# ETH3D/dataset-pipeline

Hardware: AMD Instinct MI355X
Metric: ICP correspondences/sec (higher is better)
Workload: dtype f32 (f64 accumulation); 1 GPU; ICPScanAligner 2 scans x 50000000 points, -d 0.01 (BASELINE.json configs[1] shape), one outer iteration per step; scans=2, parallelism=dp1

## Files before the change

dataset-pipeline_amd/csrc/e3d_icp.hip:

```cpp
#include <atomic>
#include <algorithm>
#include <cfloat>
#include <chrono>
#include <cmath>
#include <condition_variable>
#include <cstdio>
#include <functional>
#include <map>
#include <memory>
#include <mutex>
#include <thread>

#include "../../include/e3d_hip.h"
#include "e3d_comm.hpp"
#include "e3d_icp_kernels.hpp"
#include "e3d_math.hpp"

#pragma clang fp contract(off)

namespace e3d {

static thread_local std::string g_last_error;
void set_last_error(const std::string& msg) { g_last_error = msg; }
const char* last_error_cstr() { return g_last_error.c_str(); }

int require_device() {
  int n = 0;
  if (hipGetDeviceCount(&n) != hipSuccess || n <= 0) throw Error(E3D_ERR_NO_DEVICE, "no HIP device visible (libe3dhip needs an MI355X / gfx950 GPU)");
  return n;
}

struct IcpSwitches {
  int nn_mode = [] { const int v = env_int("E3D_NN_MODE", 0); return (v >= 0 && v <= 5) ? v : 0; }();
  int half = env_int("E3D_NN_HALF", 1);
  bool occupancy = env_default_on("E3D_NN_PRUNE");
  size_t dense_cells = [] { const char* e = getenv("E3D_DENSE_CELLS"); return e ? (size_t)strtoull(e, nullptr, 10) : (size_t)1 << 33; }();
  bool use_cert = env_default_on("E3D_NN_CERT");
  bool cert_skip = env_default_on("E3D_NN_CERT_SKIP");
  bool per_query = env_default_on("E3D_NN_PERQUERY");
  bool want_stats = env_default_off("E3D_NN_STATS");
  bool nn_profile = env_default_off("E3D_NN_PROFILE");
  double margin_frac = env_double("E3D_NN_MARGIN", 0.08), near_frac = env_double("E3D_NN_NEAR", 0.4);
  double np_frac = env_double("E3D_NN_NP_EXTRA", 0.5), np_gate = env_double("E3D_NN_NP_GATE", 0.2);
  size_t prune_min_list = (size_t)env_double("E3D_NN_PRUNE_MIN", 262144.0);
  long long far_div = [] { const char* e = getenv("E3D_NN_FAR_DIV"); return e ? atoll(e) : 32ll; }();
  bool fuse_update = env_default_on("E3D_NN_FUSE_UPDATE");
  double fuse_gate = env_double("E3D_NN_FUSE_GATE", 0.003);
  bool far_batch = env_default_on("E3D_NN_FAR_BATCH");
  bool seed_allowed = env_default_on("E3D_NN_SEED");
  double seed_frac = env_double("E3D_NN_SEED_FRAC", 0.3), seed_near = env_double("E3D_NN_SEED_NEAR", 0.4);
  bool seed_fresh = env_double("E3D_NN_SEED_FRESH", 0.0) != 0.0;
  bool batching = env_default_on("E3D_ICP_BATCH");
  int batch_mode = env_int("E3D_ICP_BATCH", 2);
  bool resident = env_default_on("E3D_ICP_RESIDENT");
  bool sequential_dsum = env_default_off("E3D_ICP_SEQUENTIAL_DISTANCE_SUM");
  bool lm_profile = env_default_off("E3D_LM_PROFILE");
  bool lm_trace = getenv("E3D_LM_TRACE") != nullptr;
  int solve_threads = env_int("E3D_LM_SOLVE_THREADS", 4);
  bool speculate = env_default_on("E3D_LM_SPECULATE");
  int spec_offset = env_int("E3D_LM_SPEC_OFFSET", 0);
};
static const IcpSwitches& icp_switches() { static const IcpSwitches sw; return sw; }

static int g_device = 0;
static int g_nn_mode = icp_switches().nn_mode;
static std::atomic<unsigned long long> g_grid_generation{0};

struct Cloud {
  size_t n = 0;
  bool fixed = false;
  DevBuf<float> raw_xyz, raw_nrm;
  float T[12] = {1, 0, 0, 0, 0, 1, 0, 0, 0, 0, 1, 0};
  bool grid_valid = false;
  float grid_radius = -1.f;
  float grid_T[12];
  DevBuf<float4> L4, LN, G4;
  DevBuf<HashEntry> table;
  DevBuf<unsigned> dense_start;
  bool has_dense = false;
  DevBuf<unsigned long long> half_prefix;
// ... 617 lines not shown
  NnPhase(hipStream_t st, int sl) : s(st), slot(sl) { if (icp_switches().nn_profile) { (void)hipStreamSynchronize(s); t0 = std::chrono::steady_clock::now(); } }
  ~NnPhase() { if (icp_switches().nn_profile) { (void)hipStreamSynchronize(s); g_nn_prof[slot] += std::chrono::duration<double, std::milli>(std::chrono::steady_clock::now() - t0).count(); } }
};
static void print_nn_profile(size_t n_pairs) {
  if (!icp_switches().nn_profile) return;
  fprintf(stderr, "[nn profile] certify + bounded search %.1f ms, keys + sort %.1f ms, match scan + compaction (+ plane growth) %.1f ms, %zu pairs\n",
          g_nn_prof[0], g_nn_prof[1], g_nn_prof[2], n_pairs);
  for (double& v : g_nn_prof) v = 0;
}

static bool pair_is_dense(const e3d_icp* h, const Cloud& tgt) {
  return h->nn_mode >= 2 || (h->nn_mode == 0 && (double)tgt.n >= 4.0 * (double)std::max(tgt.n_cells, 1u));
}
static bool pair_uses_rows(const e3d_icp* h, const Cloud& tgt) {
  return pair_is_dense(h, tgt) && tgt.has_dense && (h->nn_mode == 0 || h->nn_mode == 3 || h->nn_mode == 5);
}
static bool far_list_is_short(size_t n_far, size_t n) {
  const long long div = icp_switches().far_div;
  return n_far > 0 && (div <= 0 || n_far * (size_t)div < n);
}
static size_t resident_rows_cap(size_t n) { return div_up(n, 64) * 64; }
static size_t resident_bytes(size_t n) { return resident_rows_cap(n) * 24 + n * 4 + div_up(n, 64) * 4; }
static size_t source_view_cap(size_t n) { return resident_rows_cap(n) + 64; }
static size_t source_view_bytes(size_t n) { return source_view_cap(n) * 24; }
static bool alloc_trace() { static const bool on = [] { const char* e = getenv("E3D_ALLOC_TRACE"); return e && e[0] == '1'; }(); return on; }

struct BatchItem {
  PairJob* job; Cloud* src; Cloud* tgt; size_t j0, n; PairState* ps;
  InvMap im; CertParams cert; BoundParams bp; double cum_pair;
  MotionBound cum_up;
  float near2; bool none_near;
  bool certified = false, from_state = false; size_t n_near = 0, n_far = 0;
  bool rows_reset = false;
};

static void certify_ran(BatchItem& it, const unsigned* todo_len) {
  it.n_near = todo_len[0]; it.n_far = todo_len[1];
  it.ps->settled_frac = it.n ? 1.0 - (double)(it.n_near + it.n_far) / (double)it.n : 1.0;
  it.ps->certify_motion = it.src->last_motion + it.tgt->last_motion;
}

static void prepare_pair(BatchItem& it, float d) {
  const IcpSwitches& sw = icp_switches();
  const Cloud& src = *it.src; const Cloud& tgt = *it.tgt;
  const PairState& ps = *it.ps;
  it.im = make_invmap(tgt);
  it.cum_pair = src.cum_motion + tgt.cum_motion;
  MotionBound m_lo;
  pair_motion_bounds(ps, src, tgt, m_lo, it.cum_up);
  it.cert = make_cert_params(tgt, m_lo);
  it.n_far = it.n; it.n_near = 0;
  it.certified = !ps.fresh && sw.use_cert && certify_now(ps, src, tgt);
  it.from_state = !ps.fresh && sw.use_cert && !it.certified;
  it.near2 = (float)((sw.near_frac * (double)d) * (sw.near_frac * (double)d));
  it.none_near = sw.np_frac > 0 && (src.last_motion + tgt.last_motion) < sw.np_gate * (double)d;
  double smin = cloud_smin(tgt);
  if (!(smin > 1e-12)) smin = 1e-12;
  double m_local = 0;
  for (int k = 0; k < 3; ++k) m_local = std::max(m_local, std::max(std::fabs((double)tgt.lmin[k]), std::fabs((double)tgt.lmax[k])));
  it.bp.margin = (float)(sw.margin_frac * (double)d);
  it.bp.rho_scale = round_up_f((1.0 + 1e-5) / smin);
  it.bp.rho_pad = round_up_f(2.0 * tgt.build_slack + 8.0 * FLT_EPSILON * m_local);
  it.bp.lo = it.cert.lo;
  it.bp.cell_scale = it.cert.cell_scale; it.bp.cell_sub = it.cert.cell_sub;
  it.bp.np_extra = it.none_near ? (float)(sw.np_frac * (double)d) : 0.f;
}
// ... 6 lines not shown
  const unsigned long long* half = tgt.has_half ? tgt.half_prefix.p : nullptr;
  h->tm_bounded.start(s);
  launch_nn_bounded(srcG, todo_near, it.n_near, tgt.G4.p, tgt.dense_start.p, half, h->nn_mode == 5, tgt.grid, it.im, tgt.qrange, radius_sq(d), it.bp,
                    ps.match.p, ps.match2.p, match_d2, ps.lbe.p, s);
  if (far_list_is_short(it.n_far, it.n)) {
    launch_nn_bounded(srcG, todo_far, it.n_far, tgt.G4.p, tgt.dense_start.p, half, h->nn_mode == 5, tgt.grid, it.im, tgt.qrange, radius_sq(d), it.bp,
                      ps.match.p, ps.match2.p, match_d2, ps.lbe.p, s);
    it.n_near += it.n_far; it.n_far = 0;
  }
  h->tm_bounded.stop(s);
  if (it.n_near > 0) { rec.nn_bounded_launches++; rec.nn_bounded_queries += (long long)it.n_near; rec.nn_kernel_launches++; }
}

static void search_far_list(e3d_icp* h, BatchItem& it, const unsigned* list, float* match_d2, float d, EventTimer* nn_timer, e3d_icp_iter_record& rec) {
  hipStream_t s = h->stream;
  PairState& ps = *it.ps;
  const float4* srcG = it.src->G4.p + it.j0;
  size_t n_rows = 0;
  if (it.n_far > 0) {
    NnPhase ph(s, 1);
    n_rows = sort_query_keys_pruned(h, ps, *it.tgt, srcG, list, it.n_far, it.im, radius_sq(d), it.cert, match_d2, it.from_state);
    rec.nn_sort_calls++; rec.nn_kernel_launches++;
  }
  if (nn_timer) nn_timer->start(s);
  if (n_rows == 0) return;
  if (!nn_timer) h->tm_search.start(s);
  launch_rows(3, *it.tgt, srcG, h->vals_b.p, n_rows, it.im, radius_sq(d), it.cert, ps.match.p, match_d2, ps.lbe.p, ps.match2.p, s);
  if (!nn_timer) h->tm_search.stop(s);
  rec.nn_search_launches++; rec.nn_search_queries += (long long)n_rows; rec.nn_kernel_launches++;
}

static void print_pair_stats(const BatchItem& it) {
  if (!icp_switches().want_stats) return;
  fprintf(stderr, "[nn %d->%d] queries %zu bounded %zu rows %zu cum %.3g (last %.3g) err %.3g\n", it.job->src, it.job->tgt, it.n, it.n_near, it.n_far,
          it.cum_pair, it.src->last_motion + it.tgt->last_motion, it.src->err_max + it.tgt->err_max);
}

struct RowFrames { bool sg, tg; bool reset; };
static void ensure_source_view(Cloud& c, bool global, hipStream_t s) {
  const size_t cap = source_view_cap(c.n);
  bool valid = c.view_valid && c.V0.cap >= cap && c.V1.cap >= cap && c.view_gen == c.generation && c.view_global == global;
  if (valid && global && std::memcmp(c.view_T, c.T, sizeof c.view_T) != 0) valid = false;
  if (valid) return;
  if (alloc_trace() && (c.V0.cap < cap || c.V1.cap < cap))
    fprintf(stderr, "[rows] source view of cloud %d: %zu points, %zu bytes (%s frame)\n", c.cloud_index, c.n, source_view_bytes(c.n), global ? "global" : "local");
  c.V0.reserve(cap); c.V1.reserve(cap);
  launch_source_view(global ? c.G4.p : c.L4.p, c.LN.p, c.n, cap, global, to_affine(c.T), c.V0.p, c.V1.p, s);
  c.view_valid = true; c.view_global = global; c.view_gen = c.generation;
  std::memcpy(c.view_T, c.T, sizeof c.view_T);
}
static RowFrames ensure_resident_rows(PairState& ps, Cloud& src, const Cloud& tgt, size_t n, hipStream_t s) {
  const size_t cap = resident_rows_cap(n);
  const bool sg = src.fixed || src.cloud_index == 0, tg = tgt.fixed || tgt.cloud_index == 0;
  ensure_source_view(src, sg, s);
  bool valid = ps.rows_valid && ps.r0.cap >= cap && ps.r1.cap >= cap && ps.src_global == sg && ps.tgt_global == tg;
  if (valid && sg && std::memcmp(ps.src_T, src.T, sizeof ps.src_T) != 0) valid = false;
  if (valid && tg && std::memcmp(ps.tgt_T, tgt.T, sizeof ps.tgt_T) != 0) valid = false;
  if (!valid) {
    ps.r0.reserve(cap); ps.r1.reserve(cap); ps.plane_match.reserve(n); ps.glist.reserve(div_up(n, 64));
    E3D_HIP(hipMemsetAsync(ps.plane_match.p, 0xFE, sizeof(int) * n, s));
    if (cap > n) {
      E3D_HIP(hipMemsetAsync(ps.r0.p + n, 0xFF, sizeof(float2) * (cap - n), s));
      E3D_HIP(hipMemsetAsync(ps.r1.p + n, 0, sizeof(float4) * (cap - n), s));
    }
    ps.src_global = sg; ps.tgt_global = tg;
    std::memcpy(ps.src_T, src.T, sizeof ps.src_T); std::memcpy(ps.tgt_T, tgt.T, sizeof ps.tgt_T);
    ps.rows_valid = true;
  }
// ... 224 lines not shown
    prepare_pair(it, d);
    const RowFrames rf = ensure_resident_rows(ps, src, tgt, n, s);
    const bool tg = rf.tg;
    it.rows_reset = rf.reset;
    NnPairDev& P = T.pair[i];
    P.Gsrc = src.G4.p + it.j0; P.Gtgt = tgt.G4.p; P.S = tgt.dense_start.p; P.H8 = tgt.half_prefix.p;
    P.match = ps.match.p; P.match2 = ps.match2.p; P.lbe = ps.lbe.p; P.match_d2 = sl.match_d2.p;
    P.todo_near = sl.todo_near.p; P.todo_far = sl.todo_far.p; P.counts = h->d_todo_all.p + 2 * i;
    P.n = (unsigned)n; P.none_near = it.none_near ? 1 : 0;
    P.cum_up = it.cum_up; P.near2 = it.near2;
    P.g = tgt.grid; P.im = it.im; P.qr = tgt.qrange; P.bp = it.bp;
    P.Ptgt = tg ? tgt.G4.p : tgt.L4.p; P.LNtgt = tgt.LN.p;
    P.tgt_global = tg ? 1 : 0; P.Ttgt = to_affine(tgt.T);
    P.R0 = ps.r0.p; P.R1 = ps.r1.p; P.plane_match = ps.plane_match.p; P.glist = ps.glist.p;
    if (it.certified) { cert_blocks += (unsigned)div_up(n, (size_t)kNnCertBlockQueries); cert_queries += (long long)n; }
    T.cert_end[i] = cert_blocks;
    const unsigned nb = (unsigned)div_up(n, kBlock);
    upd_blocks += nb; T.upd_end[i] = upd_blocks;
    chunks += (unsigned)div_up((size_t)nb, (size_t)kNnScanChunk); T.chunk_end[i] = chunks;
  }
  h->block_counts.reserve(upd_blocks); h->block_d2.reserve(upd_blocks); h->block_groups.reserve(upd_blocks);
  h->chunk_sum.reserve(chunks + 1); h->chunk_d2.reserve(chunks + 1); h->chunk_groups.reserve(chunks + 1); h->chunk_rewritten.reserve(chunks + 1);
  {
    if (sw.fuse_update && cert_blocks) { h->block_done.reserve(upd_blocks); E3D_HIP(hipMemsetAsync(h->block_done.p, 0, upd_blocks, s)); }
    unsigned b0 = 0;
    for (size_t i = 0; i < B; ++i) {
      NnPairDev& P = T.pair[i];
      const bool on = sw.fuse_update && cert_blocks && items[i].certified && !items[i].rows_reset && (1.0 - items[i].ps->settled_frac) < sw.fuse_gate;
      P.upd_counts = on ? h->block_counts.p + b0 : nullptr; P.upd_d2 = on ? h->block_d2.p + b0 : nullptr;
      P.upd_groups = on ? h->block_groups.p + b0 : nullptr; P.upd_done = on ? h->block_done.p + b0 : nullptr;
      b0 = T.upd_end[i];
    }
  }
  E3D_HIP(hipMemcpyAsync(h->d_batch.p, h->h_batch.p, sizeof(NnBatchDev), hipMemcpyHostToDevice, s));
  if (cert_blocks) {
    h->tm_certify.start(s);
    launch_nn_certify_multi(h->d_batch.p, cert_blocks, radius_sq(d), s);
    h->tm_certify.stop(s);
    rec.nn_certify_launches++; rec.nn_certify_queries += cert_queries; rec.nn_kernel_launches++;
    copy_out(h->h_todo_all.p, h->d_todo_all.p, 2 * sizeof(unsigned) * B, s);
  }
  sync(h);
  unsigned job_blocks = 0;
  long long job_queries = 0;
  auto add_job = [&](size_t i, const unsigned* list, size_t n_list) {
    if (!n_list) return;
    const int jb = T.n_jobs++;
    T.job_pair[jb] = (int)i; T.job_list[jb] = list; T.job_n[jb] = (unsigned)n_list;
    job_blocks += (unsigned)div_up(n_list, kBlock); T.job_end[jb] = job_blocks;
    job_queries += (long long)n_list;
  };
  for (size_t i = 0; i < B; ++i) {
    BatchItem& it = items[i];
    if (!it.certified) continue;
    e3d_icp::PairSlot& sl = *h->slots[i];
    certify_ran(it, h->h_todo_all.p + 2 * i);
    add_job(i, sl.todo_near.p, it.n_near);
    if (far_list_is_short(it.n_far, it.n)) {
      add_job(i, sl.todo_far.p, it.n_far);
      it.n_near += it.n_far; it.n_far = 0;
    }
  }
  auto launch_bounded_jobs = [&] {
    if (T.n_jobs <= 0) return;
    E3D_HIP(hipMemcpyAsync(h->d_batch.p, h->h_batch.p, sizeof(NnBatchDev), hipMemcpyHostToDevice, s));
    h->tm_bounded.start(s);
    launch_nn_bounded_half_multi(h->d_batch.p, job_blocks, radius_sq(d), s);
    h->tm_bounded.stop(s);
    rec.nn_bounded_launches++; rec.nn_bounded_queries += job_queries; rec.nn_kernel_launches++;
  };
  auto seeds_for = [&](const BatchItem& it) { return sw.seed_allowed && it.n_far > 0 && (it.ps->fresh ? sw.seed_fresh : it.ps->matched_frac >= sw.seed_frac); };
  size_t far_pairs = 0, far_total = 0;
  int kb_max = 1;
  for (size_t i = 0; i < B; ++i) if (items[i].n_far > 0) { ++far_pairs; far_total += items[i].n_far; kb_max = std::max(kb_max, items[i].tgt->key_bits); }
  int pair_bits = 0;
  while (((size_t)1 << pair_bits) < B) ++pair_bits;
  const bool far_multi = sw.far_batch && far_pairs > 0 && (kb_max + pair_bits <= 32 || kb_max > 31) && kb_max + pair_bits <= 63;
  if (!far_multi) launch_bounded_jobs();
  if (far_multi) {
    const bool k32 = kb_max <= 31 && kb_max + pair_bits <= 32;
    bool seed_any = false;
    for (size_t i = 0; i < B; ++i)
      if (seeds_for(items[i])) seed_any = true;
    const size_t key_block = seed_any ? (size_t)kQuerySeedBlock : (size_t)kQueryKeysBlock;
    unsigned key_blocks = 0;
    for (size_t i = 0; i < B; ++i) {
      BatchItem& it = items[i];
      NnPairDev& P = T.pair[i];
      P.far_n = 0; P.far_list = nullptr; P.far_flags = 0; P.occ = nullptr; P.occ_stride = 0; P.rows_off = 0; P.rows_n = 0; P.seed_list = nullptr; P.seed2 = 0.f;
      if (it.n_far > 0) {
// ... 932 lines not shown
```

dataset-pipeline_amd/csrc/e3d_icp_certify.hip:

```cpp
#include <cstdlib>

#include "e3d_icp_device.hpp"

#pragma clang fp contract(off)

namespace e3d {

constexpr int kCertPerWave = 512;
template <int kCertUnroll>
__device__ __forceinline__ void nn_certify_body(const unsigned bx, const float4* __restrict__ Gsrc, size_t n, const float4* __restrict__ Gtgt,
                                                const MotionBound cum_up, float r2, float near2, int none_near, int* __restrict__ match,
                                                int* __restrict__ match2, const float* __restrict__ lbe,
                                                float* __restrict__ match_d2, unsigned* __restrict__ todo_near,
                                                unsigned* __restrict__ todo_far, unsigned* __restrict__ counts,
                                                unsigned* __restrict__ upd_counts = nullptr, double* __restrict__ upd_d2 = nullptr,
                                                unsigned* __restrict__ upd_groups = nullptr, unsigned char* __restrict__ upd_done = nullptr) {
  __shared__ unsigned s_list[2][kBlock / kWave][kCertPerWave];
  __shared__ unsigned s_cnt[2][kBlock / kWave];
  __shared__ unsigned s_base[2];
  const int lane = threadIdx.x & 63, w = threadIdx.x >> 6;
  const size_t j0 = ((size_t)bx * (kBlock / kWave) + (size_t)w) * kCertPerWave;
  unsigned cn = 0, cf = 0;
  for (int step0 = 0; step0 < kCertPerWave / kWave; step0 += kCertUnroll) {
    size_t jj[kCertUnroll];
    bool vv[kCertUnroll];
    int mm[kCertUnroll], mm2[kCertUnroll];
    float ll[kCertUnroll];
    float4 qq[kCertUnroll], c1[kCertUnroll], c2v[kCertUnroll];
#pragma unroll
    for (int u = 0; u < kCertUnroll; ++u) {
      jj[u] = j0 + (size_t)(step0 + u) * kWave + (size_t)lane;
      vv[u] = jj[u] < n;
      const size_t js = vv[u] ? jj[u] : 0;
      mm[u] = ld_stream(match + js); mm2[u] = ld_stream(match2 + js); ll[u] = ld_stream(lbe + js); qq[u] = ld_stream(Gsrc + js);
    }
#pragma unroll
    for (int u = 0; u < kCertUnroll; ++u) {
      c1[u] = Gtgt[mm[u] >= 0 ? mm[u] : 0];
      c2v[u] = Gtgt[(mm[u] >= 0 && mm2[u] >= 0) ? mm2[u] : 0];
    }
    unsigned ub_c = 0, ub_g = 0, ub_gm = 0;
    double ub_t = 0.0;
    bool ub_bad = false;
    static_assert(kCertUnroll == 4, "four steps of 64 queries = one block of the row update");
#pragma unroll
    for (int u = 0; u < kCertUnroll; ++u) {
    const size_t j = jj[u];
    const bool valid = vv[u];
    bool ok = false, near = false;
    bool swapped = false;
    float v_ok = 0.f;
    if (valid) {
      const float thr = (ll[u] - motion_up(qq[u], cum_up)) * 0.999999f;
      const float lim = thr * thr * 0.999999f;
      const int m = mm[u];
      if (m >= 0) {
        const int m2 = mm2[u];
        const float4 q = qq[u];
        const float4 c = c1[u];
        float v = sqdist_l2(q.x, q.y, q.z, c.x, c.y, c.z);
        if (m2 >= 0) {
          const float4 c2 = c2v[u];
          const float v2 = sqdist_l2(q.x, q.y, q.z, c2.x, c2.y, c2.z);
          if (v2 < v || (v2 == v && __float_as_uint(c2.w) < __float_as_uint(c.w))) {
            v = v2;
            if (thr > 0.f && v < lim && v < r2) { match[j] = m2; match2[j] = m; swapped = true; }
          }
        }
        ok = (thr > 0.f) && (v < lim) && (v < r2);
        near = v < near2;
        if (ok) { st_stream(match_d2 + j, v); v_ok = v; }
      } else {
        ok = (thr > 0.f) && (lim >= r2);
        near = none_near != 0;
        st_stream(match_d2 + j, r2);
      }
    }
    const unsigned long long fn = __ballot(valid && !ok && near), ff = __ballot(valid && !ok && !near);
    const unsigned long long below = (1ull << lane) - 1ull;
    if (valid && !ok) {
      if (near) s_list[0][w][cn + (unsigned)__popcll(fn & below)] = (unsigned)j;
      else s_list[1][w][cf + (unsigned)__popcll(ff & below)] = (unsigned)j | (mm[u] < 0 ? kListNoPartner : 0u);
    }
    cn += (unsigned)__popcll(fn); cf += (unsigned)__popcll(ff);
    if (upd_done) {
      const bool f = valid && mm[u] >= 0;
      const unsigned gc = (unsigned)__popcll(__ballot(f));
      const double gd = wave_sum((f && ok) ? (double)v_ok : 0.0);
      ub_c += gc; ub_t += gd;
      if (gc) { ++ub_g; ub_gm |= 1u << u; }
      if (__ballot(valid && (!ok || swapped))) ub_bad = true;
    }
    }
    if (upd_done) {
      const size_t blk = j0 / kBlock + (size_t)(step0 / kCertUnroll);
      if (blk < (n + kBlock - 1) / kBlock && lane == 0) {
        if (!ub_bad) { upd_counts[blk] = ub_c; upd_d2[blk] = ub_t; upd_groups[blk] = ub_g | (ub_gm << 8); }
        upd_done[blk] = ub_bad ? 0 : 1;
      }
    }
  }
  if (lane == 0) { s_cnt[0][w] = cn; s_cnt[1][w] = cf; }
  __syncthreads();
  if (threadIdx.x < 2) {
    unsigned tot = 0;
    for (int k = 0; k < kBlock / kWave; ++k) tot += s_cnt[threadIdx.x][k];
    s_base[threadIdx.x] = tot ? atomicAdd(&counts[threadIdx.x], tot) : 0u;
  }
  __syncthreads();
  unsigned bn = s_base[0], bf = s_base[1];
  for (int k = 0; k < w; ++k) { bn += s_cnt[0][k]; bf += s_cnt[1][k]; }
  for (unsigned i = (unsigned)lane; i < cn; i += kWave) todo_near[bn + i] = s_list[0][w][i];
  for (unsigned i = (unsigned)lane; i < cf; i += kWave) todo_far[bf + i] = s_list[1][w][i];
}

template <int kCertUnroll>
__global__ __launch_bounds__(kBlock) void k_nn_certify(const float4* __restrict__ Gsrc, size_t n, const float4* __restrict__ Gtgt,
                                                       MotionBound cum_up, float r2, float near2, int none_near, int* __restrict__ match,
                                                       int* __restrict__ match2, const float* __restrict__ lbe,
                                                       float* __restrict__ match_d2, unsigned* __restrict__ todo_near,
                                                       unsigned* __restrict__ todo_far, unsigned* __restrict__ counts) {
  nn_certify_body<kCertUnroll>(blockIdx.x, Gsrc, n, Gtgt, cum_up, r2, near2, none_near, match, match2, lbe, match_d2, todo_near, todo_far, counts);
}

__global__ __launch_bounds__(kBlock) void k_nn_certify_multi(const NnBatchDev* __restrict__ B, float r2) {
  const int p = nn_find_range(B->cert_end, B->n_pairs, blockIdx.x);
  const unsigned bx = blockIdx.x - (p ? B->cert_end[p - 1] : 0u);
  const NnPairDev& P = B->pair[p];
  nn_certify_body<4>(bx, P.Gsrc, (size_t)P.n, P.Gtgt, P.cum_up, r2, P.near2, P.none_near, P.match, P.match2, P.lbe, P.match_d2,
                     P.todo_near, P.todo_far, P.counts, P.upd_counts, P.upd_d2, P.upd_groups, P.upd_done);
}

template <int LPQ>
__global__ __launch_bounds__(kBlock) void k_nn_bounded(const float4* __restrict__ Gsrc, const unsigned* __restrict__ list,
                                                       unsigned n_list, const float4* __restrict__ Gtgt, const unsigned* __restrict__ S,
                                                       GridDesc g, InvMap im, QueryRange qr, float r2, BoundParams bp,
                                                       int* __restrict__ match, int* __restrict__ match2,
                                                       float* __restrict__ match_d2, float* __restrict__ lbe) {
  const unsigned i = (blockIdx.x * blockDim.x + threadIdx.x) / LPQ;
  const int sub = threadIdx.x % LPQ;
  if (i >= n_list) return;
  const unsigned j = list[i] & kListIndexMask;
  const float4 q = Gsrc[j];
  const int m = match[j];
  float d1 = r2;
  if (m >= 0) {
// ... 73 lines not shown
  }
  if (sub != 0) return;
  tie = (bd == bd2 && bd < kInf) || (bd2 == b3 && bd2 < kInf);
  if (tie) {
    bd = kInf; bd2 = kInf; b3 = kInf; bpos = -1; bpos2 = -1;
    unsigned boi = 0u, boi2 = 0u;
    for (int cz = z0; cz <= z1; ++cz) {
      for (int cy = y0; cy <= y1; ++cy) {
        const size_t row = ((size_t)cz * qr.D[1] + (size_t)cy) * qr.D[0];
        const unsigned s0 = S[row + (size_t)x0], s1 = S[row + (size_t)x1 + 1];
        for (unsigned p = s0; p < s1; ++p) {
          const float4 c = Gtgt[p];
          const float d2 = sqdist_l2(q.x, q.y, q.z, c.x, c.y, c.z);
          const unsigned oi = __float_as_uint(c.w);
          if (d2 < bd || (d2 == bd && oi < boi)) {
            b3 = fminf(b3, bd2); bd2 = bd; boi2 = boi; bpos2 = bpos; bd = d2; boi = oi; bpos = (int)p;
          } else if (d2 < bd2 || (d2 == bd2 && oi < boi2)) {
            b3 = fminf(b3, bd2); bd2 = d2; boi2 = oi; bpos2 = (int)p;
          } else {
            b3 = fminf(b3, d2);
          }
        }
      }
    }
  }
  const bool has1 = bd < r2, has2 = bd2 < r2;
  match[j] = has1 ? bpos : -1;
  match2[j] = has2 ? bpos2 : -1;
  match_d2[j] = has1 ? bd : r2;
  const float others2 = has2 ? b3 : (has1 ? bd2 : bd);
  lbe[j] = sqrtf(fminf(others2, cover_all2)) * 0.999999f + motion_lo(q, bp.lo);
}

constexpr int kHalfRuns = 18;
template <int BATCH>
__device__ __forceinline__ void nn_bounded_half_body(const unsigned bx, const float4* __restrict__ Gsrc, const unsigned* __restrict__ list,
                                                     unsigned n_list, const float4* __restrict__ Gtgt, const unsigned* __restrict__ S,
                                                     const unsigned long long* __restrict__ H8,
                                                     const GridDesc& g, const InvMap& im, const QueryRange& qr, float r2, const BoundParams& bp,
                                                     int* __restrict__ match, int* __restrict__ match2,
                                                     float* __restrict__ match_d2, float* __restrict__ lbe) {
  __shared__ unsigned s_runs[kHalfRuns][kBlock];
  __shared__ unsigned char s_len[kHalfRuns][kBlock];
  const unsigned i = bx * blockDim.x + threadIdx.x;
  if (i >= n_list) return;
  const unsigned j = list[i] & kListIndexMask;
  const float4 q = Gsrc[j];
  const int m = match[j];
  float d1 = r2;
  if (m >= 0) {
    const float4 pc = Gtgt[m];
    d1 = sqdist_l2(q.x, q.y, q.z, pc.x, pc.y, pc.z);
    const int m2 = match2[j];
    if (m2 >= 0) { const float4 pc2 = Gtgt[m2]; d1 = fminf(d1, sqdist_l2(q.x, q.y, q.z, pc2.x, pc2.y, pc2.z)); }
  }
  const float dr = sqrtf(fminf(d1, r2)) + ((m < 0) ? bp.np_extra : bp.margin);
  const float cover2 = (d1 < r2) ? fminf(dr * dr * 1.000001f, r2) : ((m < 0) ? dr * dr * 1.000001f : r2);
  const float rho = sqrtf(cover2) * bp.rho_scale + bp.rho_pad;
  const float dx = q.x - im.t[0], dy = q.y - im.t[1], dz = q.z - im.t[2];
  const float lx = im.Linv[0] * dx + im.Linv[1] * dy + im.Linv[2] * dz;
  const float ly = im.Linv[3] * dx + im.Linv[4] * dy + im.Linv[5] * dz;
  const float lz = im.Linv[6] * dx + im.Linv[7] * dy + im.Linv[8] * dz;
  const float inv_h = 2.f * g.inv_cell;
  const int NX = 2 * (int)qr.D[0], NY = 2 * (int)qr.D[1], NZ = 2 * (int)qr.D[2];
  const int FX0 = max(cell_coord(lx - rho, g.origin[0], inv_h) - 2 * qr.lo[0], 0), FX1 = min(cell_coord(lx + rho, g.origin[0], inv_h) - 2 * qr.lo[0], NX - 1);
  const int FY0 = max(cell_coord(ly - rho, g.origin[1], inv_h) - 2 * qr.lo[1], 0), FY1 = min(cell_coord(ly + rho, g.origin[1], inv_h) - 2 * qr.lo[1], NY - 1);
  const int FZ0 = max(cell_coord(lz - rho, g.origin[2], inv_h) - 2 * qr.lo[2], 0), FZ1 = min(cell_coord(lz + rho, g.origin[2], inv_h) - 2 * qr.lo[2], NZ - 1);
  const float kInf = __uint_as_float(0x7f800000u);
  float cover_box2 = 0.f;
  const bool any = FX0 <= FX1 && FY0 <= FY1 && FZ0 <= FZ1;
  if (any) {
    const float ux = (lx - g.origin[0]) * inv_h - (float)(2 * qr.lo[0]), uy = (ly - g.origin[1]) * inv_h - (float)(2 * qr.lo[1]),
                uz = (lz - g.origin[2]) * inv_h - (float)(2 * qr.lo[2]);
    float fd = kInf;
    if (FX0 > 0) fd = fminf(fd, ux - (float)FX0);
    if (FX1 < NX - 1) fd = fminf(fd, (float)(FX1 + 1) - ux);
    if (FY0 > 0) fd = fminf(fd, uy - (float)FY0);
    if (FY1 < NY - 1) fd = fminf(fd, (float)(FY1 + 1) - uy);
    if (FZ0 > 0) fd = fminf(fd, uz - (float)FZ0);
    if (FZ1 < NZ - 1) fd = fminf(fd, (float)(FZ1 + 1) - uz);
    fd = fminf(fd, 8.0f);
    const float cb = fd * (bp.cell_scale * 0.5f) - bp.cell_sub;
    cover_box2 = cb > 0.f ? cb * cb : 0.f;
  }
  const float cover_all2 = fmaxf(cover2, cover_box2);
  float bd = kInf, bd2 = kInf, b3 = kInf;
  int bpos = -1, bpos2 = -1;
  const int cx0 = FX0 >> 1, cx1 = FX1 >> 1;
  int nr = 0;
#define RUN_S(i) s_runs[(i)][threadIdx.x]
#define RUN_LEN(i) s_len[(i)][threadIdx.x]
#define RUN_E(i) (RUN_S(i) + (unsigned)RUN_LEN(i))
  if (any) {
    const int nz = FZ1 - FZ0 + 1, ny = FY1 - FY0 + 1, nx = cx1 - cx0 + 1;
    if (nz <= 3 && ny <= 3 && nx <= 2) {
      const int gz0 = FZ0 >> 1, gy0 = FY0 >> 1;
      unsigned cs[8];
      unsigned long long ce[8];
#pragma unroll
      for (int t = 0; t < 8; ++t) {
        const int gz = min(gz0 + (t >> 2), FZ1 >> 1), gy = min(gy0 + ((t >> 1) & 1), FY1 >> 1), cx = min(cx0 + (t & 1), cx1);
        const size_t lin = ((size_t)gz * qr.D[1] + (size_t)gy) * qr.D[0] + (size_t)cx;
        cs[t] = S[lin];
        ce[t] = H8[lin];
      }
      const int dz = (FZ1 >> 1) - gz0, dy = (FY1 >> 1) - gy0, dxc = cx1 - cx0;
      bool dense = false;
#pragma unroll
      for (int t = 0; t < 8; ++t)
        dense = dense || ((t >> 2) <= dz && ((t >> 1) & 1) <= dy && (t & 1) <= dxc && ce[t] == ~0ull);
      if (dense) {
        nr = -1;
      } else {
#pragma unroll
        for (int t = 0; t < 8; ++t) {
          if ((t >> 2) <= dz && ((t >> 1) & 1) <= dy && (t & 1) <= dxc) {
            const int cz2 = 2 * (gz0 + (t >> 2)), cy2 = 2 * (gy0 + ((t >> 1) & 1)), cx2 = 2 * (cx0 + (t & 1));
            const bool xa = FX0 > cx2, xb = FX1 > cx2;
            const unsigned st = cs[t], lo = (unsigned)ce[t], hi = (unsigned)(ce[t] >> 32);
#pragma unroll
            for (int zz = 0; zz < 2; ++zz)
#pragma unroll
              for (int yy = 0; yy < 2; ++yy) {
                if (cz2 + zz >= FZ0 && cz2 + zz <= FZ1 && cy2 + yy >= FY0 && cy2 + yy <= FY1) {
// ... 75 lines not shown
    auto exact_run = [&](unsigned s0, unsigned s1) {
      for (unsigned p = s0; p < s1; ++p) {
        const float4 c = Gtgt[p];
        const float d2 = sqdist_l2(q.x, q.y, q.z, c.x, c.y, c.z);
        const unsigned oi = __float_as_uint(c.w);
        if (d2 < bd || (d2 == bd && oi < boi)) {
          b3 = fminf(b3, bd2); bd2 = bd; boi2 = boi; bpos2 = bpos; bd = d2; boi = oi; bpos = (int)p;
        } else if (d2 < bd2 || (d2 == bd2 && oi < boi2)) {
          b3 = fminf(b3, bd2); bd2 = d2; boi2 = oi; bpos2 = (int)p;
        } else {
          b3 = fminf(b3, d2);
        }
      }
    };
    if (nr >= 0) {
      for (int r = 0; r < nr; ++r) exact_run(RUN_S(r), RUN_E(r));
    } else {
      for (int gz = FZ0 >> 1; gz <= (FZ1 >> 1); ++gz)
        for (int gy = FY0 >> 1; gy <= (FY1 >> 1); ++gy) {
          const size_t row = ((size_t)gz * qr.D[1] + (size_t)gy) * qr.D[0];
          exact_run(S[row + (size_t)cx0], S[row + (size_t)cx1 + 1]);
        }
    }
  }
#undef RUN_S
#undef RUN_E
#undef RUN_LEN
  const bool has1 = bd < r2, has2 = bd2 < r2;
  match[j] = has1 ? bpos : -1;
  match2[j] = has2 ? bpos2 : -1;
  match_d2[j] = has1 ? bd : r2;
  const float others2 = has2 ? b3 : (has1 ? bd2 : bd);
  lbe[j] = sqrtf(fminf(others2, cover_all2)) * 0.999999f + motion_lo(q, bp.lo);
}

template <int BATCH>
__global__ __launch_bounds__(kBlock) void k_nn_bounded_half(const float4* __restrict__ Gsrc, const unsigned* __restrict__ list,
                                                            unsigned n_list, const float4* __restrict__ Gtgt, const unsigned* __restrict__ S,
                                                            const unsigned long long* __restrict__ H8,
                                                            GridDesc g, InvMap im, QueryRange qr, float r2, BoundParams bp,
                                                            int* __restrict__ match, int* __restrict__ match2,
                                                            float* __restrict__ match_d2, float* __restrict__ lbe) {
  nn_bounded_half_body<BATCH>(blockIdx.x, Gsrc, list, n_list, Gtgt, S, H8, g, im, qr, r2, bp, match, match2, match_d2, lbe);
}

__global__ __launch_bounds__(kBlock) void k_nn_bounded_half_multi(const NnBatchDev* __restrict__ B, float r2) {
  const int jb = nn_find_range(B->job_end, B->n_jobs, blockIdx.x);
  const unsigned bx = blockIdx.x - (jb ? B->job_end[jb - 1] : 0u);
  const int p = __builtin_amdgcn_readfirstlane(B->job_pair[jb]);
  const NnPairDev& P = B->pair[p];
  const GridDesc g = P.g; const InvMap im = P.im; const QueryRange qr = P.qr; const BoundParams bp = P.bp;
  nn_bounded_half_body<8>(bx, P.Gsrc, B->job_list[jb], B->job_n[jb], P.Gtgt, P.S, P.H8, g, im, qr, r2, bp, P.match, P.match2,
                          P.match_d2, P.lbe);
}

constexpr int kSeedPerThread = 4;
static_assert((unsigned)(kBlock * kSeedPerThread) == kQuerySeedBlock, "queries per block of the seeding key kernel");
template <typename KeyT, int kSeedProbes>
__global__ __launch_bounds__(kBlock) void k_query_seed_multi(const NnBatchDev* __restrict__ B, float r2, KeyT* __restrict__ keys, unsigned* __restrict__ vals,
                                                             unsigned* __restrict__ counts) {
  __shared__ unsigned s_cnt[2][kBlock / kWave][kSeedPerThread];
  __shared__ unsigned s_base[2];
  const int p = nn_find_range(B->far_end, B->n_pairs, blockIdx.x);
  const unsigned bx = blockIdx.x - (p ? B->far_end[p - 1] : 0u);
  const NnPairDev& P = B->pair[p];
  const GridDesc g = P.g; const InvMap im = P.im; const QueryRange qr = P.qr;
// ... 150 lines not shown
}

void launch_nn_certify(const float4* Gsrc, size_t n, const float4* Gtgt, const MotionBound& cum_up, float r2, float near2, bool none_near, int* match, int* match2,
                       const float* lbe, float* match_d2, unsigned* todo_near, unsigned* todo_far, unsigned* counts, hipStream_t s) {
  if (!n) return;
  hipLaunchKernelGGL(k_nn_certify<4>, dim3((unsigned)div_up(n, (size_t)kCertPerWave * (kBlock / kWave))), dim3(kBlock), 0, s, Gsrc, n, Gtgt,
                     cum_up, r2, near2, none_near ? 1 : 0, match, match2, lbe, match_d2, todo_near, todo_far, counts);
}

void launch_nn_bounded(const float4* Gsrc, const unsigned* list, size_t n_list, const float4* Gtgt, const unsigned* dense_start,
                       const unsigned long long* half_prefix, bool half_always, const GridDesc& g, const InvMap& im, const QueryRange& qr, float r2,
                       const BoundParams& bp, int* match, int* match2, float* match_d2, float* lbe, hipStream_t s) {
  if (!n_list) return;
  static const size_t quad_limit = [] { const char* e = getenv("E3D_NN_QUAD_LIMIT"); return e ? (size_t)atoll(e) : (size_t)12000000; }();
  static const size_t half_min = [] { const char* e = getenv("E3D_NN_HALF_MIN"); return e ? (size_t)atoll(e) : (size_t)200000; }();
  if (half_prefix && (half_always || n_list >= half_min)) {
    hipLaunchKernelGGL((k_nn_bounded_half<8>), dim3((unsigned)div_up(n_list, kBlock)), dim3(kBlock), 0, s, Gsrc, list, (unsigned)n_list,
                       Gtgt, dense_start, half_prefix, g, im, qr, r2, bp, match, match2, match_d2, lbe);
    return;
  }
  if (n_list <= quad_limit)
    hipLaunchKernelGGL(k_nn_bounded<4>, dim3((unsigned)div_up(4 * n_list, kBlock)), dim3(kBlock), 0, s, Gsrc, list, (unsigned)n_list, Gtgt,
                       dense_start, g, im, qr, r2, bp, match, match2, match_d2, lbe);
  else
    hipLaunchKernelGGL(k_nn_bounded<1>, dim3((unsigned)div_up(n_list, kBlock)), dim3(kBlock), 0, s, Gsrc, list, (unsigned)n_list, Gtgt,
                       dense_start, g, im, qr, r2, bp, match, match2, match_d2, lbe);
}

void launch_nn_certify_multi(const NnBatchDev* batch, unsigned n_blocks, float r2, hipStream_t s) {
  static_assert(kNnCertBlockQueries == kCertPerWave * (kBlock / kWave), "queries per certificate block");
  if (!n_blocks) return;
  hipLaunchKernelGGL(k_nn_certify_multi, dim3(n_blocks), dim3(kBlock), 0, s, batch, r2);
}
void launch_nn_bounded_half_multi(const NnBatchDev* batch, unsigned n_blocks, float r2, hipStream_t s) {
  if (!n_blocks) return;
  hipLaunchKernelGGL(k_nn_bounded_half_multi, dim3(n_blocks), dim3(kBlock), 0, s, batch, r2);
}

void launch_query_seed_multi(bool keys32, const NnBatchDev* batch, unsigned n_blocks, float r2, void* keys, unsigned* vals, unsigned* counts, hipStream_t s) {
  if (!n_blocks) return;
  static const int probes = [] { const char* e = getenv("E3D_NN_SEED_PROBES"); return e ? atoi(e) : 8; }();
  if (probes == 4) {
    if (keys32) hipLaunchKernelGGL((k_query_seed_multi<unsigned, 4>), dim3(n_blocks), dim3(kBlock), 0, s, batch, r2, (unsigned*)keys, vals, counts);
    else hipLaunchKernelGGL((k_query_seed_multi<unsigned long long, 4>), dim3(n_blocks), dim3(kBlock), 0, s, batch, r2, (unsigned long long*)keys, vals, counts);
  } else {
    if (keys32) hipLaunchKernelGGL((k_query_seed_multi<unsigned, 8>), dim3(n_blocks), dim3(kBlock), 0, s, batch, r2, (unsigned*)keys, vals, counts);
    else hipLaunchKernelGGL((k_query_seed_multi<unsigned long long, 8>), dim3(n_blocks), dim3(kBlock), 0, s, batch, r2, (unsigned long long*)keys, vals, counts);
  }
}

}
```

dataset-pipeline_amd/csrc/e3d_icp_kernels.hpp:

```cpp
#pragma once

#include "e3d_grid.hpp"

namespace e3d {

enum { kModeCost = 0,
       kModeOne = 1,
       kModeTwo = 2,
       kModeTwoCross = 3
};
constexpr int kLmMaxPoses = 10;
constexpr int kLmSlot = 91;
constexpr int kRowCap = 128;
constexpr unsigned kListNoPartner = 0x80000000u, kListIndexMask = 0x7FFFFFFFu;
constexpr int kRowSpan = 4;
constexpr int kNNCap = 256;

struct LmSet {
  const float4 *A, *B, *C;
  const float2 *V1, *R0;
  const unsigned* glist;
  long long n;
  int block_begin, nblocks;
  int mode;
// ... 45 lines not shown
  float rho_scale;
  float rho_pad;
  MotionBound lo;
  float cell_scale, cell_sub;
  float np_extra;
};
void launch_nn_bounded(const float4* Gsrc, const unsigned* list, size_t n_list, const float4* Gtgt, const unsigned* dense_start,
                       const unsigned long long* half_prefix, bool half_always, const GridDesc& g, const InvMap& im, const QueryRange& qr, float r2,
                       const BoundParams& bp, int* match, int* match2, float* match_d2, float* lbe, hipStream_t s);
constexpr int kNnBatchPairs = 32;
constexpr int kNnBatchJobs = 2 * kNnBatchPairs;
struct NnPairDev {
  const float4* Gsrc;
  const float4* Gtgt;
  const unsigned* S;
  const unsigned long long* H8;
  int *match, *match2;
  float* lbe;
  float* match_d2;
  unsigned *todo_near, *todo_far;
  unsigned* counts;
  unsigned n;
  int none_near;
  MotionBound cum_up;
  float near2;
  GridDesc g; InvMap im; QueryRange qr; BoundParams bp;
  const float4 *Ptgt, *LNtgt;
  int tgt_global;
  Affine Ttgt;
  float2* R0; float4* R1;
  int* plane_match;
  unsigned* glist;
  unsigned* upd_counts; double* upd_d2; unsigned* upd_groups; unsigned char* upd_done;
  const unsigned* far_list;
  const unsigned* occ;
  unsigned far_n, occ_stride;
  int far_flags;
  unsigned rows_off, rows_n;
  unsigned* seed_list;
  float seed2;
};
constexpr unsigned kQueryKeysBlock = 2048;
constexpr unsigned kQuerySeedBlock = 1024;
struct NnBatchDev {
  int n_pairs, n_jobs;
  int key_shift;
  unsigned far_end[kNnBatchPairs];
  unsigned rows_end[kNnBatchPairs];
  unsigned cert_end[kNnBatchPairs];
  unsigned upd_end[kNnBatchPairs];
  unsigned chunk_end[kNnBatchPairs];
  unsigned job_end[kNnBatchJobs];
  int job_pair[kNnBatchJobs];
  unsigned job_n[kNnBatchJobs];
  const unsigned* job_list[kNnBatchJobs];
  NnPairDev pair[kNnBatchPairs];
};
void launch_nn_certify_multi(const NnBatchDev* batch, unsigned n_blocks, float r2, hipStream_t s);
void launch_nn_bounded_half_multi(const NnBatchDev* batch, unsigned n_blocks, float r2, hipStream_t s);
void launch_query_keys_multi(bool keys32, const NnBatchDev* batch, unsigned n_blocks, float r2, void* keys, unsigned* vals, unsigned* counts, hipStream_t s);
void launch_query_seed_multi(bool keys32, const NnBatchDev* batch, unsigned n_blocks, float r2, void* keys, unsigned* vals, unsigned* counts, hipStream_t s);
void launch_nn_rows_multi(const NnBatchDev* batch, unsigned n_blocks, const unsigned* order, float r2, hipStream_t s);
void launch_corr_update_multi(const NnBatchDev* batch, unsigned n_blocks, unsigned* block_counts, double* block_d2, unsigned* block_groups, hipStream_t s);
void launch_corr_totals_multi(const NnBatchDev* batch, int n_pairs, unsigned n_chunks, const unsigned* block_counts, const double* block_d2,
                              const unsigned* block_groups, unsigned long long* chunk_sum, double* chunk_d2, unsigned* chunk_groups,
                              unsigned* chunk_rewritten, unsigned long long* totals, double* total_d2, hipStream_t s);
constexpr int kNnCertBlockQueries = 2048;
constexpr int kNnScanChunk = 256;
void launch_half_keys(const float* xyz, size_t n, const GridDesc& g, unsigned* keys, unsigned* vals, hipStream_t s);
void launch_cell_keys_ordered(const float* xyz, const unsigned* order, size_t n, const GridDesc& g, unsigned long long* keys, hipStream_t s);
void launch_half_prefix(const unsigned long long* keys, const float4* L4, size_t n, const GridDesc& g, const QueryRange& qr,
                        const unsigned* dense_start, unsigned long long* half_prefix, hipStream_t s);
struct MfParams { float S, r2s, eta2, delta4, delta4sq; };
bool mfma_filter_params(double cell, double sigma_max, int row_span, float r2, MfParams* P);
void launch_nn_mfma(const float4* Gsrc, const unsigned* order, size_t n, const float4* Gtgt, const unsigned* dense_start,
                    const GridDesc& g, const InvMap& im, const QueryRange& qr, float r2, const MfParams& P, int* match_pos,
                    float* match_d2, hipStream_t s);
int nn_row_span();
void launch_dense_counts(const unsigned long long* keys, size_t n, const QueryRange& qr, unsigned* counts, hipStream_t s);
void launch_compact_corr(const int* match_pos, const unsigned* order, size_t n, const unsigned* block_offsets, const float4* Gsrc,
                         const float4* LNsrc, const Affine& Tsrc, const float4* Gtgt, const float4* LNtgt,
                         const Affine& Ttgt, float4* A, float4* B, float4* C, size_t out_base, hipStream_t s);
void launch_gather_corr(const float* sxyz, const float* snrm, const float* txyz, const float* tnrm, const int* iq,
                        const int* im, size_t n, float4* A, float4* B, float4* C, hipStream_t s);
void launch_unpermute_matches(const int* match_pos, const float* match_d2, const unsigned* order, size_t n, const float4* Gsrc,
                              const float4* Gtgt, int* out_idx, float* out_d2, hipStream_t s);
void launch_match_d2_by_original(const int* match_pos, const float* match_d2, const unsigned* order, size_t n, const float4* Gsrc, float* out,
                                 hipStream_t s);
void launch_lm_pass(int mode, const LmSet* sets, const int* block_set, int block_base, int nblocks, double* partial, hipStream_t s);
void launch_lm_cost_multi(const LmSet* sets, const LmPose* poses, int n_sets, int n_poses, const int* block_set, int nblocks,
                          double* partial, hipStream_t s);
void launch_source_view(const float4* P, const float4* LN, size_t n, size_t cap, bool global, const Affine& T, float4* V0, float2* V1, hipStream_t s);
// ... 10 lines not shown
```

Measured before the change: 6.880 billion correspondences/s.

## Fuse bounded near-query search into the certify kernel for partially settled pairs

Adds a fused certify+bounded-search kernel. Near queries that fail certification are stored as 16-bit offsets in LDS and searched right after certification by the same wave, using a per-wave run table. This removes the todo_near list write-back and the separate bounded-half launch when a pair's unsettled fraction lies between configurable gates (default 0.02 to 0.5). The trade-off is more LDS use and a larger kernel, which may reduce occupancy, and the extra search work can load-imbalance waves.

```diff
diff --git a/dataset-pipeline_amd/csrc/e3d_icp.hip b/dataset-pipeline_amd/csrc/e3d_icp.hip
--- a/dataset-pipeline_amd/csrc/e3d_icp.hip
+++ b/dataset-pipeline_amd/csrc/e3d_icp.hip
@@ -5,6 +5,7 @@
 #include <cmath>
 #include <condition_variable>
 #include <cstdio>
+#include <cstring>
 #include <functional>
 #include <map>
 #include <memory>
@@ -28,6 +29,12 @@
   int n = 0;
   if (hipGetDeviceCount(&n) != hipSuccess || n <= 0) throw Error(E3D_ERR_NO_DEVICE, "no HIP device visible (libe3dhip needs an MI355X / gfx950 GPU)");
   return n;
+}
+
+static double env_field(const char* name, int k, double dflt) {
+  const char* e = getenv(name);
+  for (; e && k > 0; --k) { e = strchr(e, ','); if (e) ++e; }
+  return e ? atof(e) : dflt;
 }
 
 struct IcpSwitches {
@@ -46,6 +53,9 @@
   long long far_div = [] { const char* e = getenv("E3D_NN_FAR_DIV"); return e ? atoll(e) : 32ll; }();
   bool fuse_update = env_default_on("E3D_NN_FUSE_UPDATE");
   double fuse_gate = env_double("E3D_NN_FUSE_GATE", 0.003);
+  bool fuse_bounded = env_default_on("E3D_NN_FUSE_BOUNDED");
+  double fuse_bounded_lo = env_field("E3D_NN_FUSE_BOUNDED", 1, 0.02);
+  double fuse_bounded_hi = env_field("E3D_NN_FUSE_BOUNDED", 2, env_field("E3D_NN_FUSE_BOUNDED", 1, -1.0) >= 0.0 ? 1.0 : 0.5);
   bool far_batch = env_default_on("E3D_NN_FAR_BATCH");
   bool seed_allowed = env_default_on("E3D_NN_SEED");
   double seed_frac = env_double("E3D_NN_SEED_FRAC", 0.3), seed_near = env_double("E3D_NN_SEED_NEAR", 0.4);
@@ -729,6 +739,7 @@
   float near2; bool none_near;
   bool certified = false, from_state = false; size_t n_near = 0, n_far = 0;
   bool rows_reset = false;
+  size_t n_fused = 0;
 };
 
 static void certify_ran(BatchItem& it, const unsigned* todo_len) {
@@ -801,8 +812,8 @@
 
 static void print_pair_stats(const BatchItem& it) {
   if (!icp_switches().want_stats) return;
-  fprintf(stderr, "[nn %d->%d] queries %zu bounded %zu rows %zu cum %.3g (last %.3g) err %.3g\n", it.job->src, it.job->tgt, it.n, it.n_near, it.n_far,
-          it.cum_pair, it.src->last_motion + it.tgt->last_motion, it.src->err_max + it.tgt->err_max);
+  fprintf(stderr, "[nn %d->%d] queries %zu bounded %zu rows %zu cum %.3g (last %.3g) err %.3g fused %zu\n", it.job->src, it.job->tgt, it.n, it.n_near, it.n_far,
+          it.cum_pair, it.src->last_motion + it.tgt->last_motion, it.src->err_max + it.tgt->err_max, it.n_fused);
 }
 
 struct RowFrames { bool sg, tg; bool reset; };
@@ -1093,10 +1104,18 @@
       b0 = T.upd_end[i];
     }
   }
+  bool fuse_any = false;
+  for (size_t i = 0; i < B; ++i) {
+    const bool on = sw.fuse_bounded && items[i].certified && (1.0 - items[i].ps->settled_frac) >= sw.fuse_bounded_lo &&
+                    (1.0 - items[i].ps->settled_frac) <= sw.fuse_bounded_hi;
+    T.pair[i].fuse_bounded = on ? 1 : 0;
+    fuse_any = fuse_any || on;
+  }
   E3D_HIP(hipMemcpyAsync(h->d_batch.p, h->h_batch.p, sizeof(NnBatchDev), hipMemcpyHostToDevice, s));
   if (cert_blocks) {
     h->tm_certify.start(s);
-    launch_nn_certify_multi(h->d_batch.p, cert_blocks, radius_sq(d), s);
+    if (fuse_any) launch_nn_certify_bounded_multi(h->d_batch.p, cert_blocks, radius_sq(d), s);
+    else launch_nn_certify_multi(h->d_batch.p, cert_blocks, radius_sq(d), s);
     h->tm_certify.stop(s);
     rec.nn_certify_launches++; rec.nn_certify_queries += cert_queries; rec.nn_kernel_launches++;
     copy_out(h->h_todo_all.p, h->d_todo_all.p, 2 * sizeof(unsigned) * B, s);
@@ -1116,7 +1135,8 @@
     if (!it.certified) continue;
     e3d_icp::PairSlot& sl = *h->slots[i];
     certify_ran(it, h->h_todo_all.p + 2 * i);
-    add_job(i, sl.todo_near.p, it.n_near);
+    if (T.pair[i].fuse_bounded) { it.n_fused = it.n_near; rec.nn_bounded_queries += (long long)it.n_near; }
+    else add_job(i, sl.todo_near.p, it.n_near);
     if (far_list_is_short(it.n_far, it.n)) {
       add_job(i, sl.todo_far.p, it.n_far);
       it.n_near += it.n_far; it.n_far = 0;
diff --git a/dataset-pipeline_amd/csrc/e3d_icp_certify.hip b/dataset-pipeline_amd/csrc/e3d_icp_certify.hip
--- a/dataset-pipeline_amd/csrc/e3d_icp_certify.hip
+++ b/dataset-pipeline_amd/csrc/e3d_icp_certify.hip
@@ -7,19 +7,36 @@
 namespace e3d {
 
 constexpr int kCertPerWave = 512;
-template <int kCertUnroll>
+template <bool kFused> struct CertLbePtr { using type = const float* __restrict__; };
+template <> struct CertLbePtr<true> { using type = float*; };
+constexpr int kHalfRuns = 18;
+constexpr int kFusedWaveBytes = kHalfRuns * kWave * 5;
+template <bool kFused> struct CertLds { unsigned list[2][kBlock / kWave][kCertPerWave]; };
+template <> struct CertLds<true> {
+  unsigned short near[kBlock / kWave][kCertPerWave];
+  alignas(16) unsigned char tab[(kBlock / kWave) * kFusedWaveBytes];
+};
+static_assert(kFusedWaveBytes >= kCertPerWave * (int)sizeof(unsigned) && kFusedWaveBytes % 16 == 0, "a wave's far list fits its run table");
+__device__ __forceinline__ void nn_certify_search_near(const NnPairDev* __restrict__ F, int* match, int* match2, float* match_d2, float* lbe,
+                                                       unsigned j0, const unsigned short* near_w, unsigned cn, unsigned char* tab_w, int lane, float r2);
+template <int kCertUnroll, bool kFused = false>
 __device__ __forceinline__ void nn_certify_body(const unsigned bx, const float4* __restrict__ Gsrc, size_t n, const float4* __restrict__ Gtgt,
                                                 const MotionBound cum_up, float r2, float near2, int none_near, int* __restrict__ match,
-                                                int* __restrict__ match2, const float* __restrict__ lbe,
+                                                int* __restrict__ match2, typename CertLbePtr<kFused>::type lbe,
                                                 float* __restrict__ match_d2, unsigned* __restrict__ todo_near,
                                                 unsigned* __restrict__ todo_far, unsigned* __restrict__ counts,
                                                 unsigned* __restrict__ upd_counts = nullptr, double* __restrict__ upd_d2 = nullptr,
-                                                unsigned* __restrict__ upd_groups = nullptr, unsigned char* __restrict__ upd_done = nullptr) {
-  __shared__ unsigned s_list[2][kBlock / kWave][kCertPerWave];
+                                                unsigned* __restrict__ upd_groups = nullptr, unsigned char* __restrict__ upd_done = nullptr,
+                                                const NnPairDev* __restrict__ F = nullptr) {
+  __shared__ CertLds<kFused> s_lds;
   __shared__ unsigned s_cnt[2][kBlock / kWave];
   __shared__ unsigned s_base[2];
   const int lane = threadIdx.x & 63, w = threadIdx.x >> 6;
   const size_t j0 = ((size_t)bx * (kBlock / kWave) + (size_t)w) * kCertPerWave;
+  unsigned* far_w;
+  if constexpr (kFused) far_w = reinterpret_cast<unsigned*>(s_lds.tab + w * kFusedWaveBytes);
+  else far_w = s_lds.list[1][w];
+  const bool fused = kFused && F != nullptr;
   unsigned cn = 0, cf = 0;
   for (int step0 = 0; step0 < kCertPerWave / kWave; step0 += kCertUnroll) {
     size_t jj[kCertUnroll];
@@ -73,14 +90,18 @@
       } else {
         ok = (thr > 0.f) && (lim >= r2);
         near = none_near != 0;
-        st_stream(match_d2 + j, r2);
+        if (!(fused && !ok && near)) st_stream(match_d2 + j, r2);
       }
     }
     const unsigned long long fn = __ballot(valid && !ok && near), ff = __ballot(valid && !ok && !near);
     const unsigned long long below = (1ull << lane) - 1ull;
     if (valid && !ok) {
-      if (near) s_list[0][w][cn + (unsigned)__popcll(fn & below)] = (unsigned)j;
-      else s_list[1][w][cf + (unsigned)__popcll(ff & below)] = (unsigned)j | (mm[u] < 0 ? kListNoPartner : 0u);
+      if (near) {
+        if constexpr (kFused) s_lds.near[w][cn + (unsigned)__popcll(fn & below)] = (unsigned short)(j - j0);
+        else s_lds.list[0][w][cn + (unsigned)__popcll(fn & below)] = (unsigned)j;
+      } else {
+        far_w[cf + (unsigned)__popcll(ff & below)] = (unsigned)j | (mm[u] < 0 ? kListNoPartner : 0u);
+      }
     }
     cn += (unsigned)__popcll(fn); cf += (unsigned)__popcll(ff);
     if (upd_done) {
@@ -110,8 +131,16 @@
   __syncthreads();
   unsigned bn = s_base[0], bf = s_base[1];
   for (int k = 0; k < w; ++k) { bn += s_cnt[0][k]; bf += s_cnt[1][k]; }
-  for (unsigned i = (unsigned)lane; i < cn; i += kWave) todo_near[bn + i] = s_list[0][w][i];
-  for (unsigned i = (unsigned)lane; i < cf; i += kWave) todo_far[bf + i] = s_list[1][w][i];
+  if constexpr (kFused) {
+    if (!fused)
+      for (unsigned i = (unsigned)lane; i < cn; i += kWave) todo_near[bn + i] = (unsigned)j0 + (unsigned)s_lds.near[w][i];
+  } else {
+    for (unsigned i = (unsigned)lane; i < cn; i += kWave) todo_near[bn + i] = s_lds.list[0][w][i];
+  }
+  for (unsigned i = (unsigned)lane; i < cf; i += kWave) todo_far[bf + i] = far_w[i];
+  if constexpr (kFused) {
+    if (fused) nn_certify_search_near(F, match, match2, match_d2, lbe, (unsigned)j0, s_lds.near[w], cn, s_lds.tab + w * kFusedWaveBytes, lane, r2);
+  }
 }
 
 template <int kCertUnroll>
@@ -251,21 +280,10 @@
   lbe[j] = sqrtf(fminf(others2, cover_all2)) * 0.999999f + motion_lo(q, bp.lo);
 }
 
-constexpr int kHalfRuns = 18;
-template <int BATCH>
-__device__ __forceinline__ void nn_bounded_half_body(const unsigned bx, const float4* __restrict__ Gsrc, const unsigned* __restrict__ list,
-                                                     unsigned n_list, const float4* __restrict__ Gtgt, const unsigned* __restrict__ S,
-                                                     const unsigned long long* __restrict__ H8,
-                                                     const GridDesc& g, const InvMap& im, const QueryRange& qr, float r2, const BoundParams& bp,
-                                                     int* __restrict__ match, int* __restrict__ match2,
-                                                     float* __restrict__ match_d2, float* __restrict__ lbe) {
-  __shared__ unsigned s_runs[kHalfRuns][kBlock];
-  __shared__ unsigned char s_len[kHalfRuns][kBlock];
-  const unsigned i = bx * blockDim.x + threadIdx.x;
-  if (i >= n_list) return;
-  const unsigned j = list[i] & kListIndexMask;
-  const float4 q = Gsrc[j];
-  const int m = match[j];
+__device__ __forceinline__ float nn_bounded_fetch(const unsigned j, const float4* __restrict__ Gsrc, const float4* __restrict__ Gtgt,
+                                                  const int* match, const int* match2, float r2, float4& q, int& m) {
+  q = Gsrc[j];
+  m = match[j];
   float d1 = r2;
   if (m >= 0) {
     const float4 pc = Gtgt[m];
@@ -273,6 +291,15 @@
     const int m2 = match2[j];
     if (m2 >= 0) { const float4 pc2 = Gtgt[m2]; d1 = fminf(d1, sqdist_l2(q.x, q.y, q.z, pc2.x, pc2.y, pc2.z)); }
   }
+  return d1;
+}
+
+template <int BATCH, int STRIDE>
+__device__ __forceinline__ void nn_bounded_half_search(const unsigned j, const float4 q, const int m, const float d1, unsigned* runs,
+                                                       unsigned char* lens, const float4* __restrict__ Gtgt, const unsigned* __restrict__ S,
+                                                       const unsigned long long* __restrict__ H8,
+                                                       const GridDesc& g, const InvMap& im, const QueryRange& qr, float r2, const BoundParams& bp,
+                                                       int* match, int* match2, float* match_d2, float* lbe) {
   const float dr = sqrtf(fminf(d1, r2)) + ((m < 0) ? bp.np_extra : bp.margin);
   const float cover2 = (d1 < r2) ? fminf(dr * dr * 1.000001f, r2) : ((m < 0) ? dr * dr * 1.000001f : r2);
   const float rho = sqrtf(cover2) * bp.rho_scale + bp.rho_pad;
@@ -307,8 +334,8 @@
   int bpos = -1, bpos2 = -1;
   const int cx0 = FX0 >> 1, cx1 = FX1 >> 1;
   int nr = 0;
-#define RUN_S(i) s_runs[(i)][threadIdx.x]
-#define RUN_LEN(i) s_len[(i)][threadIdx.x]
+#define RUN_S(i) runs[(i) * STRIDE]
+#define RUN_LEN(i) lens[(i) * STRIDE]
 #define RUN_E(i) (RUN_S(i) + (unsigned)RUN_LEN(i))
   if (any) {
     const int nz = FZ1 - FZ0 + 1, ny = FY1 - FY0 + 1, nx = cx1 - cx0 + 1;
@@ -450,6 +477,52 @@
   match_d2[j] = has1 ? bd : r2;
   const float others2 = has2 ? b3 : (has1 ? bd2 : bd);
   lbe[j] = sqrtf(fminf(others2, cover_all2)) * 0.999999f + motion_lo(q, bp.lo);
+}
+
+template <int BATCH>
+__device__ __forceinline__ void nn_bounded_half_body(const unsigned bx, const float4* __restrict__ Gsrc, const unsigned* __restrict__ list,
+                                                     unsigned n_list, const float4* __restrict__ Gtgt, const unsigned* __restrict__ S,
+                                                     const unsigned long long* __restrict__ H8,
+                                                     const GridDesc& g, const InvMap& im, const QueryRange& qr, float r2, const BoundParams& bp,
+                                                     int* __restrict__ match, int* __restrict__ match2,
+                                                     float* __restrict__ match_d2, float* __restrict__ lbe) {
+  __shared__ unsigned s_runs[kHalfRuns][kBlock];
+  __shared__ unsigned char s_len[kHalfRuns][kBlock];
+  const unsigned i = bx * blockDim.x + threadIdx.x;
+  if (i >= n_list) return;
+  const unsigned j = list[i] & kListIndexMask;
+  float4 q;
+  int m;
+  const float d1 = nn_bounded_fetch(j, Gsrc, Gtgt, match, match2, r2, q, m);
+  nn_bounded_half_search<BATCH, kBlock>(j, q, m, d1, &s_runs[0][threadIdx.x], &s_len[0][threadIdx.x], Gtgt, S, H8, g, im, qr, r2, bp, match, match2,
+                                        match_d2, lbe);
+}
+
+__device__ __forceinline__ void nn_certify_search_near(const NnPairDev* __restrict__ F, int* match, int* match2, float* match_d2, float* lbe,
+                                                       unsigned j0, const unsigned short* near_w, unsigned cn, unsigned char* tab_w, int lane, float r2) {
+  const GridDesc g = F->g; const InvMap im = F->im; const QueryRange qr = F->qr; const BoundParams bp = F->bp;
+  const float4* __restrict__ Gsrc = F->Gsrc; const float4* __restrict__ Gtgt = F->Gtgt;
+  unsigned* runs = reinterpret_cast<unsigned*>(tab_w) + lane;
+  unsigned char* lens = tab_w + kHalfRuns * kWave * sizeof(unsigned) + lane;
+  for (unsigned i0 = 0; i0 < cn; i0 += kWave) {
+    const unsigned i = i0 + (unsigned)lane;
+    if (i < cn) {
+      const unsigned j = j0 + (unsigned)near_w[i];
+      float4 q;
+      int m;
+      const float d1 = nn_bounded_fetch(j, Gsrc, Gtgt, match, match2, r2, q, m);
+      nn_bounded_half_search<8, kWave>(j, q, m, d1, runs, lens, Gtgt, F->S, F->H8, g, im, qr, r2, bp, match, match2, match_d2, lbe);
+    }
+  }
+}
+
+__global__ __launch_bounds__(kBlock) void k_nn_certify_bounded_multi(const NnBatchDev* __restrict__ B, float r2) {
+  const int p = nn_find_range(B->cert_end, B->n_pairs, blockIdx.x);
+  const unsigned bx = blockIdx.x - (p ? B->cert_end[p - 1] : 0u);
+  const NnPairDev& P = B->pair[p];
+  const bool fuse = __builtin_amdgcn_readfirstlane(P.fuse_bounded) != 0;
+  nn_certify_body<4, true>(bx, P.Gsrc, (size_t)P.n, P.Gtgt, P.cum_up, r2, P.near2, P.none_near, P.match, P.match2, P.lbe, P.match_d2,
+                           P.todo_near, P.todo_far, P.counts, P.upd_counts, P.upd_d2, P.upd_groups, P.upd_done, fuse ? &P : nullptr);
 }
 
 template <int BATCH>
@@ -666,6 +739,10 @@
   if (!n_blocks) return;
   hipLaunchKernelGGL(k_nn_certify_multi, dim3(n_blocks), dim3(kBlock), 0, s, batch, r2);
 }
+void launch_nn_certify_bounded_multi(const NnBatchDev* batch, unsigned n_blocks, float r2, hipStream_t s) {
+  if (!n_blocks) return;
+  hipLaunchKernelGGL(k_nn_certify_bounded_multi, dim3(n_blocks), dim3(kBlock), 0, s, batch, r2);
+}
 void launch_nn_bounded_half_multi(const NnBatchDev* batch, unsigned n_blocks, float r2, hipStream_t s) {
   if (!n_blocks) return;
   hipLaunchKernelGGL(k_nn_bounded_half_multi, dim3(n_blocks), dim3(kBlock), 0, s, batch, r2);
diff --git a/dataset-pipeline_amd/csrc/e3d_icp_kernels.hpp b/dataset-pipeline_amd/csrc/e3d_icp_kernels.hpp
--- a/dataset-pipeline_amd/csrc/e3d_icp_kernels.hpp
+++ b/dataset-pipeline_amd/csrc/e3d_icp_kernels.hpp
@@ -101,6 +101,7 @@
   int* plane_match;
   unsigned* glist;
   unsigned* upd_counts; double* upd_d2; unsigned* upd_groups; unsigned char* upd_done;
+  int fuse_bounded;
   const unsigned* far_list;
   const unsigned* occ;
   unsigned far_n, occ_stride;
@@ -127,6 +128,7 @@
 };
 void launch_nn_certify_multi(const NnBatchDev* batch, unsigned n_blocks, float r2, hipStream_t s);
 void launch_nn_bounded_half_multi(const NnBatchDev* batch, unsigned n_blocks, float r2, hipStream_t s);
+void launch_nn_certify_bounded_multi(const NnBatchDev* batch, unsigned n_blocks, float r2, hipStream_t s);
 void launch_query_keys_multi(bool keys32, const NnBatchDev* batch, unsigned n_blocks, float r2, void* keys, unsigned* vals, unsigned* counts, hipStream_t s);
 void launch_query_seed_multi(bool keys32, const NnBatchDev* batch, unsigned n_blocks, float r2, void* keys, unsigned* vals, unsigned* counts, hipStream_t s);
 void launch_nn_rows_multi(const NnBatchDev* batch, unsigned n_blocks, const unsigned* order, float r2, hipStream_t s);
```

Result: slower. 6.112 billion correspondences/s (-11.2%).
